# millardjn/rusty_sr

Hardware: AMD Instinct MI355X
Metric: output megapixels/sec at 3x upscale (BASELINE '4x'; reference factor is hard-wired 3) (higher is better)
Workload: dtype f32

## Files before the change

rusty_sr_amd/csrc/sr_kernels.hip:

```cpp
#include <hip/hip_runtime.h>
#include <stddef.h>
#include <stdint.h>

#include <mutex>
#include <set>
#include <type_traits>
#include <utility>

#include "sr_kernels.h"

#pragma clang fp contract(off)

typedef float f32x2 __attribute__((ext_vector_type(2)));
struct f32p { float x, y; };
__device__ __forceinline__ f32p operator+(f32p a, f32p b) { return f32p{a.x + b.x, a.y + b.y}; }
__device__ __forceinline__ f32p operator-(f32p a, f32p b) { return f32p{a.x - b.x, a.y - b.y}; }
__device__ __forceinline__ f32p operator*(f32p a, f32p b) { return f32p{a.x * b.x, a.y * b.y}; }
__device__ __forceinline__ f32p p_fma(f32p a, f32p b, f32p c) { return f32p{__builtin_fmaf(a.x, b.x, c.x), __builtin_fmaf(a.y, b.y, c.y)}; }
__device__ __forceinline__ void store_map8(char* p, uint32_t a, uint32_t b) { *(uint2*)p = make_uint2(a, b); }
typedef float f32x4 __attribute__((ext_vector_type(4)));
typedef float f32x16 __attribute__((ext_vector_type(16)));
typedef _Float16 f16x8 __attribute__((ext_vector_type(8)));
typedef _Float16 f16x2 __attribute__((ext_vector_type(2)));

template <int PREC>
constexpr bool kPlanar = PREC == 1;
template <int PREC, bool FINAL>
constexpr bool kH16 = PREC == 1 && !FINAL;

namespace {

constexpr int kThreads = 256;
constexpr int kTW = 32;
constexpr int kChunkFloats = 1024;
constexpr int kRingSlots = 5;
constexpr int kRingAhead = 4;
constexpr int kRingBytes = kRingSlots * 4096;

__device__ __forceinline__ float belu(float v, float beta) {
    return __fadd_rn(__fadd_rn(__fmul_rn(beta, v), __builtin_amdgcn_sqrtf(__fadd_rn(__fmul_rn(v, v), 1.0f))), -1.0f);
}

__device__ __forceinline__ f32x2 belu2(f32x2 v, float beta) {
    const f32x2 one = {1.0f, 1.0f};
    const f32x2 t = v * v + one;
    const f32x2 s = {__builtin_amdgcn_sqrtf(t.x), __builtin_amdgcn_sqrtf(t.y)};
    const f32x2 b = {beta, beta};
    return (b * v + s) - one;
}

__device__ __forceinline__ f32p split_value(f32p accm, f32p accx) {
    return p_fma(accx, f32p{1.0f / 2048.0f, 1.0f / 2048.0f}, accm);
}
__device__ __forceinline__ f32p belu2_fused2(f32p v, f32p beta) {
    const f32p one = {1.0f, 1.0f};
    const f32p t = p_fma(v, v, one);
    const f32p s = {__builtin_amdgcn_sqrtf(t.x), __builtin_amdgcn_sqrtf(t.y)};
    return p_fma(beta, v, s) - one;
}

__device__ __forceinline__ void store_belu_tile(float* base, const f32x16& acc, float bias, float beta) {
#pragma unroll
    for (int r = 0; r < 16; r += 2) {
        const f32x2 bb = {bias, bias};
        const f32x2 o = belu2(f32x2{acc[r], acc[r + 1]} + bb, beta);
        const int row = (r & 3) + 8 * (r >> 2);
        base[row * 32] = o.x;
        base[(row + 1) * 32] = o.y;
    }
}

__device__ __forceinline__ void store_belu_tile_lds(float* grow, float* stage, const f32x16& acc, float bias, float beta, int lane) {
    float* sp = stage + (4 * (lane >> 5)) * 32 + (lane & 31);
#pragma unroll
    for (int r = 0; r < 16; r += 2) {
        const f32x2 bb = {bias, bias};
        const f32x2 o = belu2(f32x2{acc[r], acc[r + 1]} + bb, beta);
        const int row = (r & 3) + 8 * (r >> 2);
        sp[row * 32] = o.x;
        sp[(row + 1) * 32] = o.y;
    }
    const f32x4* lp = (const f32x4*)stage + lane;
    const f32x4 v0 = lp[0], v1 = lp[64], v2 = lp[128], v3 = lp[192];
    f32x4* gp = (f32x4*)grow + lane;
    gp[0] = v0; gp[64] = v1; gp[128] = v2; gp[192] = v3;
}

__device__ __forceinline__ int xcd_remap(int bid, int nblk) {
    const int q = nblk >> 3, r = nblk & 7, xcd = bid & 7, idx = bid >> 3;
    return (xcd < r ? xcd * (q + 1) : r * (q + 1) + (xcd - r) * q) + idx;
}

__device__ __forceinline__ int tile_div(int t, TileDiv d) {
    return (int)((__umulhi((uint32_t)t, d.m) + (uint32_t)t) >> d.s);
}

__device__ __forceinline__ void tile_coords(const TileGrid& g, int tiles_x, int t, int& n, int& tx, int& ty) {
    const int tpi = tiles_x * g.tiles_y;
    n = tile_div(t, g.div_tpi);
    const int r = t - n * tpi;
    if (g.bw == 0) {
        ty = tile_div(r, g.div_tx);
        tx = r - ty * tiles_x;
    } else {
        int b = tile_div(r, g.div_blk);
        if (b > g.nfull) b = g.nfull;
        const int rr = r - b * g.bw * g.tiles_y;
        const bool full = b < g.nfull;
        const int w = full ? g.bw : tiles_x - g.nfull * g.bw;
        ty = full ? tile_div(rr, g.div_bw) : tile_div(rr, g.div_rem);
        tx = b * g.bw + (rr - ty * w);
    }
}

__device__ __forceinline__ float load_img(const void* img, int img_ch, bool u8, size_t px, int c) {
    if (u8) return __fdiv_rn((float)((const uint8_t*)img)[px * img_ch + c], 255.0f);
    return ((const float*)img)[px * 3 + c];
}

constexpr float kLoScale = 2048.0f;
typedef __fp16 fp16x2_t __attribute__((ext_vector_type(2)));

__device__ __forceinline__ void split_half2(f32p v, uint32_t& hi2, uint32_t& lo2) {
    const fp16x2_t h = __builtin_amdgcn_cvt_pkrtz(v.x, v.y);
    const f32p hf = {(float)h.x, (float)h.y};
    const f32p r = (v - hf) * f32p{kLoScale, kLoScale};
    hi2 = __builtin_bit_cast(uint32_t, h);
    lo2 = __builtin_bit_cast(uint32_t, __builtin_amdgcn_cvt_pkrtz(r.x, r.y));
}

typedef unsigned short u16x2 __attribute__((ext_vector_type(2)));
__device__ __forceinline__ void domain_track(uint32_t& dom, uint32_t hi2) {
    dom = __builtin_bit_cast(uint32_t, __builtin_elementwise_max(__builtin_bit_cast(u16x2, dom), __builtin_bit_cast(u16x2, hi2 & 0x7fff7fffu)));
}
__device__ __forceinline__ void domain_report(uint32_t dom, int* flag) {
    if (((dom & 0xffffu) >= 0x7bffu) | ((dom >> 16) >= 0x7bffu)) *(volatile int*)flag = 1;
}

__device__ __forceinline__ void store_belu_tile_split_cr(char* base, const f32x16& accm, const f32x16& accx, const f32x4 (&beta)[4], bool write,
                                                         long group_stride, long lo_off, uint32_t& dom) {
#pragma unroll
    for (int j = 0; j < 4; ++j) {
        const int r = 4 * j;
        const f32p v01 = belu2_fused2(split_value(f32p{accm[r], accm[r + 1]}, f32p{accx[r], accx[r + 1]}), f32p{beta[j][0], beta[j][1]});
        const f32p v23 = belu2_fused2(split_value(f32p{accm[r + 2], accm[r + 3]}, f32p{accx[r + 2], accx[r + 3]}), f32p{beta[j][2], beta[j][3]});
        uint32_t h01, l01, h23, l23;
        split_half2(v01, h01, l01);
        split_half2(v23, h23, l23);
        domain_track(dom, h01);
        domain_track(dom, h23);
        if (write) {
            store_map8(base + j * group_stride, h01, h23);
            store_map8(base + j * group_stride + lo_off, l01, l23);
        }
    }
}

template <typename F>
__device__ __forceinline__ void for_each_acc_row(F&& f) {
#pragma unroll
    for (int r = 0; r < 16; ++r) f(r, (r & 3) + 8 * (r >> 2));
}

}

__device__ __forceinline__ const char* uniform_ptr(const void* p) {
    const uint64_t v = (uint64_t)(uintptr_t)p;
    const uint32_t lo = __builtin_amdgcn_readfirstlane((uint32_t)v), hi = __builtin_amdgcn_readfirstlane((uint32_t)(v >> 32));
    return (const char*)(uintptr_t)(((uint64_t)hi << 32) | lo);
}

template <int TH, bool IMG_U8>
__global__ __launch_bounds__(kThreads, 2) void conv0_kernel(Conv0Args a) {
    constexpr int T = TH / 4;
    constexpr int TWH = kTW + 4, THH = TH + 4, NPIX = THH * TWH;
    __shared__ __attribute__((aligned(16))) float s_x[NPIX * 3 + 16];
    __shared__ __attribute__((aligned(16))) float s_w[5 * 8 * 64];

    const int tid = threadIdx.x, lane = tid & 63;
    const int wave = __builtin_amdgcn_readfirstlane(tid >> 6);
    const int i = lane & 31, h = lane >> 5;
    const int tiles_per_img = a.tiles_x * a.tiles_y;
    for (int k = tid; k < 5 * 8 * 64; k += kThreads) s_w[k] = a.wpack[k];
    if (tid < 16) s_x[NPIX * 3 + tid] = 0.f;
    if (blockIdx.x == 0 && tid < 40) a.queue_reset[tid] = (a.queue_grid[tid >> 3] - (tid & 7) + 7) >> 3;
    __shared__ float s_lut[256];
    if constexpr (IMG_U8) s_lut[tid] = __fdiv_rn((float)tid, 255.0f);
    const float bias = a.bias[i], beta = a.beta[i];
  for (int bid = blockIdx.x; bid < a.n_tiles; bid += gridDim.x) {
    const int n = tile_div(bid, a.div_tpi), t = bid - n * tiles_per_img;
// ... 1236 lines not shown
    f32x16 wacc[NWACC];
#pragma unroll
    for (int p = 0; p < NWACC; ++p)
#pragma unroll
        for (int r = 0; r < 16; ++r) wacc[p][r] = 0.f;
    int gtap = 0, slot = 0;
    auto taps = [&](auto ks_tag) {
        constexpr int KS = decltype(ks_tag)::value;
        if constexpr (WINO) {
            using G = TileGeom<TH, KS>;
            RingStream sm{ring, a.wpack, gtap, slot, NTAPS, wave, lane};
#pragma unroll 1
            for (int half = 0; half < 2; ++half) {
                if constexpr (KS == KS0) half_steps_wino<G::TWH, G::PLANE, T>(wacc, tile + half * 4 * G::PLANE, ring, sm, wave, lane);
                else half_steps_pairs<G::TWH, G::PLANE, T>(wacc, tile + half * 4 * G::PLANE, ring, sm, wave, lane);
            }
        } else if constexpr (H16) source_steps_h16<TH, KS, T>(qm, qx, tile, ring, a.wpack, gtap, slot, NTAPS, wave, lane);
        else source_steps<TH, KS, T, NTN, PREC>(acc, accx, tile, ring, a.wpack, gtap, slot, NTAPS, wave, lane);
    };
    ring_barrier<0>();
    __builtin_amdgcn_s_setprio(0);
    taps(std::integral_constant<int, KS0>{});
    if constexpr (NSRC >= 2) {
        __builtin_amdgcn_s_setprio(3);
        stage_tile<TH, 3, PREC, NW>(tile, a.src[1], off3, a.img_stride, a.pitch, n, y0, x0, wave, lane);
        ring_barrier<0>();
        __builtin_amdgcn_s_setprio(0);
        taps(std::integral_constant<int, 3>{});
    }
    if constexpr (NSRC >= 3) {
        __builtin_amdgcn_s_setprio(3);
        stage_tile<TH, 3, PREC, NW>(tile, a.src[2], off3, a.img_stride, a.pitch, n, y0, x0, wave, lane);
        ring_barrier<0>();
        __builtin_amdgcn_s_setprio(0);
        taps(std::integral_constant<int, 3>{});
    }
    __builtin_amdgcn_s_setprio(3);
    if constexpr (FINAL)
        lin_taps<TH, T, IMG_U8, NW * 64, NTN, PREC, FACTOR>(acc, accx, tile, ring, a, a.wpack + (size_t)NTAPS * kChunkFloats, n, y0, x0, wave, lane, tid);
    uint32_t dom = 0;
    if constexpr (WINO) {
        stage_epilogue_wino<T, NWACC>(a, wacc, bias[0], beta, n, x0, y0, wave, lane, nullptr);
    } else if constexpr (H16) {
        stage_epilogue_h16<T>(a, qm, qx, beta2, n, x0, y0, wave, lane, dom);
    } else if constexpr (FINAL && PREC == 1) {
        f32x4 fbias[NTN][4];
#pragma unroll
        for (int nt = 0; nt < NTN; ++nt)
#pragma unroll
            for (int k = 0; k < 4; ++k) fbias[nt][k] = *(const f32x4*)(a.bias + 32 * nt + 16 * (lane >> 5) + 4 * k);
        stage_epilogue_final_t<T, NTN, OUT_U8, FACTOR>(a, acc, accx, fbias, n, x0, y0, wave, lane);
    } else {
        static_assert(PREC == 0, "the split-half mode's tiles have epilogues of their own");
        stage_epilogue<TH, T, NTN, FINAL, OUT_U8, FACTOR>(a, acc, bias, beta, n, x0, y0, wave, lane);
    }
    if constexpr (PREC == 1 && !FINAL) domain_report(dom, a.domain);
}

#define SR_WAIT_ROW(k, extra) "s_waitcnt vmcnt(" #k ")" extra "\n\ts_branch .Lsrwait%=\n\t"
#define SR_WAIT_ROWS10(b, extra)                                                                                              \
    SR_WAIT_ROW(b##0, extra) SR_WAIT_ROW(b##1, extra) SR_WAIT_ROW(b##2, extra) SR_WAIT_ROW(b##3, extra) SR_WAIT_ROW(b##4, extra) \
    SR_WAIT_ROW(b##5, extra) SR_WAIT_ROW(b##6, extra) SR_WAIT_ROW(b##7, extra) SR_WAIT_ROW(b##8, extra) SR_WAIT_ROW(b##9, extra)
#define SR_WAIT_JUMP(maxn)                                                                                                   \
    "s_max_i32 %0, %1, 0\n\ts_min_i32 %0, %0, " #maxn "\n\ts_lshl_b32 %0, %0, 3\n\ts_add_u32 %0, %0, 12\n\t"                 \
    "s_getpc_b64 vcc\n\ts_add_u32 vcc_lo, vcc_lo, %0\n\ts_addc_u32 vcc_hi, vcc_hi, 0\n\ts_setpc_b64 vcc\n\t"
#define SR_WAIT_TABLE(extra)                                                                                                \
    SR_WAIT_JUMP(15) SR_WAIT_ROWS10(, extra) SR_WAIT_ROW(10, extra) SR_WAIT_ROW(11, extra) SR_WAIT_ROW(12, extra)               \
    SR_WAIT_ROW(13, extra) SR_WAIT_ROW(14, extra) SR_WAIT_ROW(15, extra) ".Lsrwait%=:"
#define SR_WAIT_TABLE64(extra)                                                                                              \
    SR_WAIT_JUMP(63) SR_WAIT_ROWS10(, extra) SR_WAIT_ROWS10(1, extra) SR_WAIT_ROWS10(2, extra) SR_WAIT_ROWS10(3, extra)         \
    SR_WAIT_ROWS10(4, extra) SR_WAIT_ROWS10(5, extra) SR_WAIT_ROW(60, extra) SR_WAIT_ROW(61, extra) SR_WAIT_ROW(62, extra)      \
    SR_WAIT_ROW(63, extra) ".Lsrwait%=:"
template <bool LGKM, bool WIDE = false>
__device__ __forceinline__ void wait_vm_n(int pending) {
    if (__builtin_constant_p(pending)) {
        switch (pending < 0 ? 0 : pending) {
#define SR_CASE(k) case k: if constexpr (LGKM) asm volatile("s_waitcnt vmcnt(" #k ") lgkmcnt(0)" ::: "memory"); else asm volatile("s_waitcnt vmcnt(" #k ")" ::: "memory"); break;
            SR_CASE(0) SR_CASE(1) SR_CASE(2) SR_CASE(3) SR_CASE(4) SR_CASE(5) SR_CASE(6) SR_CASE(7) SR_CASE(8) SR_CASE(9) SR_CASE(10)
            SR_CASE(11) SR_CASE(12) SR_CASE(13) SR_CASE(14)
#undef SR_CASE
            default: if constexpr (LGKM) asm volatile("s_waitcnt vmcnt(15) lgkmcnt(0)" ::: "memory"); else asm volatile("s_waitcnt vmcnt(15)" ::: "memory"); break;
        }
        return;
    }
    const int p = __builtin_amdgcn_readfirstlane(pending);
    int t;
    if constexpr (WIDE) {
        if constexpr (LGKM) asm volatile(SR_WAIT_TABLE64(" lgkmcnt(0)") : "=&s"(t) : "s"(p) : "vcc", "scc", "memory");
        else asm volatile(SR_WAIT_TABLE64("") : "=&s"(t) : "s"(p) : "vcc", "scc", "memory");
    } else {
        if constexpr (LGKM) asm volatile(SR_WAIT_TABLE(" lgkmcnt(0)") : "=&s"(t) : "s"(p) : "vcc", "scc", "memory");
        else asm volatile(SR_WAIT_TABLE("") : "=&s"(t) : "s"(p) : "vcc", "scc", "memory");
    }
}
template <bool LGKM, bool WIDE = false>
__device__ __forceinline__ void wait_vm_barrier(int pending) {
    wait_vm_n<LGKM, WIDE>(pending);
    __builtin_amdgcn_s_barrier();
    asm volatile("" ::: "memory");
}

template <int KS>
struct HalfTile {
    using G = TileGeom<8, KS>;
    static constexpr int NG_SMALL = TileGeom<4, KS>::NG;
    static constexpr int BYTES = 4 * G::PLANE;
    static constexpr int STEPS = (KS * KS + 1) / 2;
    static_assert(TileGeom<4, KS>::TWH == G::TWH, "a small tile is the top of a big one");
    uint32_t off[G::NG];
    template <int PREC>
    __device__ __forceinline__ void init(int pitch, int lane) {
#pragma unroll
        for (int g = 0; g < G::NG; ++g) {
            const int P = min(g * 64 + lane, G::NPIX - 1);
            const int prow = P / G::TWH, pcol = P - prow * G::TWH;
            off[g] = kPlanar<PREC> ? (uint32_t)(prow * pitch) * 128u + (uint32_t)pcol * 16u : (uint32_t)(prow * pitch + pcol) * 128u;
        }
    }
    template <int PREC>
    static __device__ __forceinline__ int chunk_of(int khalf, int wave) {
        return PREC == 0 ? 4 * khalf + wave : (wave < 2 ? 2 * khalf + wave : 4 + 2 * khalf + (wave - 2));
    }
    template <int PREC>
    __device__ __forceinline__ void stage(uint32_t buf, const float* __restrict__ src, int khalf, long img_stride, int pitch,
                                          int n, int y0, int x0, int wave) const {
        const char* origin = origin_of<PREC>(src, khalf, img_stride, pitch, n, y0, x0, wave);
        const uint32_t dst = __builtin_amdgcn_readfirstlane(buf + wave * G::PLANE);
#pragma unroll
        for (int g = 0; g < G::NG; ++g) lds_dma16<0>(origin, off[g], dst + g * 1024);
    }
    template <int PREC>
    static __device__ __forceinline__ const char* origin_of(const float* __restrict__ src, int khalf, long img_stride, int pitch, int n,
                                                            int y0, int x0, int wave) {
        if constexpr (kPlanar<PREC>)
            return uniform_ptr((const char*)(src + ((size_t)n * img_stride + (long)(y0 - G::R) * pitch) * 32) + (long)(x0 - G::R) * 16 +
                               (size_t)chunk_of<PREC>(khalf, wave) * pitch * 16);
        else
            return uniform_ptr((const char*)(src + ((size_t)n * img_stride + (long)(y0 - G::R) * pitch + (x0 - G::R)) * 32) +
                               chunk_of<PREC>(khalf, wave) * 16);
    }
    static __device__ __forceinline__ uint32_t plane_of(uint32_t buf, int wave) { return __builtin_amdgcn_readfirstlane(buf + wave * G::PLANE); }
    __device__ __forceinline__ void stage_one(int g, const char* origin, uint32_t dst) const { lds_dma16<0>(origin, off[g], dst + g * 1024); }
};

struct StepStream {
    int slot;
    int nsteps;
    bool have_next;
    int issued;
    int q[kRingAhead];
    int tile_seq;
};

__device__ __forceinline__ void step_request(StepStream& st, int gs, uint32_t ring_lds, const char* wbase, int lane) {
    int req = gs + kRingAhead;
    bool go = true;
    if (req >= st.nsteps) {
        go = st.have_next;
        req -= st.nsteps;
    }
#pragma unroll
    for (int k = 0; k + 1 < kRingAhead; ++k) st.q[k] = st.q[k + 1];
    if (go) {
        int s2 = st.slot + kRingAhead;
        if (s2 >= kRingSlots) s2 -= kRingSlots;
        lds_dma16_at(wbase, (uint32_t)req * 4096u, (uint32_t)(lane * 16), ring_lds + s2 * 4096);
        ++st.issued;
    }
    st.q[kRingAhead - 1] = st.issued;
}
template <int EXTRA>
__device__ __forceinline__ void step_advance(StepStream& st, bool tile, bool wide = false) {
    int need = st.q[EXTRA];
    if (tile && st.tile_seq > need) need = st.tile_seq;
    if (wide) wait_vm_barrier<EXTRA == 0, true>(st.issued - need);
    else wait_vm_barrier<EXTRA == 0>(st.issued - need);
    st.slot = st.slot == kRingSlots - 1 ? 0 : st.slot + 1;
}

struct HalfRequest {
    int ng;
    const char* origin;
    uint32_t dst;
};

__device__ __forceinline__ void wait_vm(int pending) { wait_vm_n<false>(pending); }

template <bool IMG_U8, int TH>
struct LinPrefetch {
    static constexpr int TWH = kTW + 2, THH = TH + 2, NPIX = THH * TWH, PER = (NPIX + 255) / 256;
    uint32_t raw[PER][3];
    int seq;
    __device__ __forceinline__ void issue(const StageArgs& a, int n, int y0, int x0, int tid, StepStream& st) {
#pragma unroll
        for (int k = 0; k < PER; ++k) {
            const int p = min(tid + 256 * k, NPIX - 1);
            const int py = p / TWH, px = p - py * TWH;
            const int gy = min(max(y0 - 1 + py, 0), a.H - 1), gx = min(max(x0 - 1 + px, 0), a.W - 1);
            const size_t gp = (size_t)n * a.H * a.W + (size_t)gy * a.W + gx;
            if constexpr (IMG_U8) {
                const uint8_t* q = (const uint8_t*)a.img + gp * a.img_ch;
                asm volatile("global_load_ubyte %0, %1, off" : "=v"(raw[k][0]) : "v"(q) : "memory");
                asm volatile("global_load_ubyte %0, %1, off offset:1" : "=v"(raw[k][1]) : "v"(q) : "memory");
                asm volatile("global_load_ubyte %0, %1, off offset:2" : "=v"(raw[k][2]) : "v"(q) : "memory");
            } else {
                const float* q = (const float*)a.img + gp * 3;
                asm volatile("global_load_dword %0, %1, off" : "=v"(raw[k][0]) : "v"(q) : "memory");
                asm volatile("global_load_dword %0, %1, off offset:4" : "=v"(raw[k][1]) : "v"(q) : "memory");
                asm volatile("global_load_dword %0, %1, off offset:8" : "=v"(raw[k][2]) : "v"(q) : "memory");
            }
        }
        st.issued += 3 * PER;
        seq = st.issued;
    }
    __device__ __forceinline__ void store_split(char* s_hi, int lo_off, const uint32_t* s_lut2, float scale, int tid, const StepStream& st) {
        wait_vm(st.issued - seq);
#pragma unroll
        for (int k = 0; k < PER; ++k)
#pragma unroll
            for (int ch = 0; ch < 3; ++ch) asm volatile("" : "+v"(raw[k][ch]));
#pragma unroll
        for (int k = 0; k < PER; ++k) {
            const int p = tid + 256 * k;
            if (p < NPIX) {
                if constexpr (IMG_U8) lin_split_store_u8(s_hi, lo_off, p, s_lut2[raw[k][0]], s_lut2[raw[k][1]], s_lut2[raw[k][2]]);
                else lin_split_store_f32(s_hi, lo_off, p, __uint_as_float(raw[k][0]), __uint_as_float(raw[k][1]), __uint_as_float(raw[k][2]), scale);
            }
        }
    }
    __device__ __forceinline__ void store(float* s_x, const float* s_lut, int tid, const StepStream& st) {
        wait_vm(st.issued - seq);
#pragma unroll
        for (int k = 0; k < PER; ++k)
#pragma unroll
            for (int ch = 0; ch < 3; ++ch) asm volatile("" : "+v"(raw[k][ch]));
#pragma unroll
        for (int k = 0; k < PER; ++k) {
            const int p = tid + 256 * k;
            if (p < NPIX) {
                f32x4 v;
                if constexpr (IMG_U8) {
                    v.x = s_lut[raw[k][0]]; v.y = s_lut[raw[k][1]]; v.z = s_lut[raw[k][2]];
                } else {
                    v.x = __uint_as_float(raw[k][0]); v.y = __uint_as_float(raw[k][1]); v.z = __uint_as_float(raw[k][2]);
                }
                v.w = 0.f;
                *(f32x4*)&s_x[p * 4] = v;
            }
        }
    }
};

struct QueueState {
    uint32_t pulled;
    uint32_t heads;
    int seq_pull, seq_snap;
    int own;
};
__device__ __forceinline__ void queue_pull_async(const StageArgs& a, int xcd, int wave, int lane, StepStream& st, QueueState& qs) {
    if (wave != 0) return;
    if (lane == 0) {
        const int* p = a.queue + xcd;
        asm volatile("global_atomic_add %0, %1, %2, off sc0" : "=v"(qs.pulled) : "v"(p), "v"(1u) : "memory");
    }
    qs.seq_pull = ++st.issued;
}
__device__ __forceinline__ void queue_presolve(const StageArgs& a, int xcd, int wave, int lane, StepStream& st, QueueState& qs) {
    if (wave != 0) return;
    wait_vm(st.issued - qs.seq_pull);
    asm volatile("" : "+v"(qs.pulled));
    const int idx = __builtin_amdgcn_readfirstlane((int)qs.pulled);
    qs.own = queue_slot(xcd, a.grid[0].ntiles, a.grid[1].ntiles, idx);
    if (qs.own < 0) {
        const int* p = a.queue + (lane & 7);
        asm volatile("global_load_dword %0, %1, off sc1" : "=v"(qs.heads) : "v"(p) : "memory");
        qs.seq_snap = ++st.issued;
    }
}
__device__ __forceinline__ void queue_publish(const StageArgs& a, int xcd, int wave, int lane, StepStream& st, QueueState& qs, volatile int* mailbox) {
    if (wave != 0) return;
    int t = qs.own;
    if (t < 0) {
        const int nbig = a.grid[0].ntiles, nsmall = a.grid[1].ntiles;
        wait_vm(st.issued - qs.seq_snap);
        asm volatile("" : "+v"(qs.heads));
        for (int k = 1; k < 8 && t < 0; ++k) {
            const int x = (xcd + k) & 7;
            if ((int)__builtin_amdgcn_readlane((int)qs.heads, x) >= queue_total(x, nbig, nsmall)) continue;
            int j = 0;
            if (lane == 0) j = atomicAdd(&a.queue[x], 1);
            t = queue_slot(x, nbig, nsmall, __builtin_amdgcn_readfirstlane(j));
        }
    }
    if (lane == 0) *mailbox = t;
    asm volatile("s_waitcnt lgkmcnt(0)" ::: "memory");
}

struct NoHook { __device__ __forceinline__ void operator()() const {} };
template <int PREC, int KSN, typename Hook = NoHook>
struct PipeStream {
    StepStream& st;
    const HalfRequest& rq;
    const HalfTile<KSN>& htn;
    const StageArgs& a;
    uint32_t ring_lds;
    const char* wbase;
    int gs0;
    int wave, lane;
    volatile int* mailbox;
    int xcd;
    QueueState& qs;
    int snap_step;
    int step_no;
    Hook last_step_hook;
    __device__ __forceinline__ void begin_step() {
        step_request(st, gs0 + step_no, ring_lds, wbase, lane);
        if (mailbox && step_no == snap_step) queue_presolve(a, xcd, wave, lane, st, qs);
        ++step_no;
    }
    __device__ __forceinline__ void piece(int g) {
        if (g < HalfTile<KSN>::G::NG && g < rq.ng) {
            htn.stage_one(g, rq.origin, rq.dst);
            st.tile_seq = ++st.issued;
        }
    }
    __device__ __forceinline__ int slot() const { return st.slot; }
    template <int EXTRA> __device__ __forceinline__ void end_step(bool last) {
        if (last) last_step_hook();
        if (last && mailbox) queue_publish(a, xcd, wave, lane, st, qs, mailbox);
        step_advance<EXTRA>(st, last, PREC == 1 && gs0 + step_no <= kRingAhead);
    }
};

template <int NSRC, int KS0, bool FINAL, bool IMG_U8, bool OUT_U8, int PREC, int FACTOR = 3, bool WINO = false>
__global__ __launch_bounds__(256, 2) void conv_stage_pipe_kernel(StageArgs a) {
    static_assert(!WINO || (NSRC <= 2 && KS0 == 5 && !FINAL && PREC == 0), "WINO: stages 1 and 2 of the exact mode");
    __builtin_amdgcn_s_setprio(3);
    constexpr int NTN = FINAL ? (FACTOR * FACTOR + 9) / 10 : 1;
    using H0 = HalfTile<KS0>;
    using H3 = HalfTile<3>;
    constexpr int HB = H0::BYTES;
    constexpr int NH = 2 * NSRC;
    constexpr bool H16 = kH16<PREC, FINAL>;
    constexpr int NSTEPS = WINO ? 2 * (kWinoSteps + (NSRC - 1) * H3::STEPS)
                         : H16 ? KS0 * KS0 + (NSRC - 1) * 9
                               : 2 * (H0::STEPS + (NSRC - 1) * H3::STEPS) * NTN;
    extern __shared__ __attribute__((aligned(16))) char smem[];
    char* ring = smem + 2 * HB;
    volatile int* s_next = (volatile int*)(ring + kRingBytes);
    float* s_wlin = (float*)(ring + kRingBytes + 16);
    float* s_lut = s_wlin + 9 * NTN * 128;
    constexpr bool kLinOwn = FINAL && NTN == 1;
    float* s_xown = s_lut + 256;
    const uint32_t lds0 = lds_addr(smem);

    const int tid = threadIdx.x, lane = tid & 63;
    const int wave = __builtin_amdgcn_readfirstlane(tid >> 6);
    const int i = lane & 31;
    const int nbig = a.grid[0].ntiles, nsmall = a.grid[1].ntiles;
    const int xcd = blockIdx.x & 7;
    const uint32_t ring_lds = __builtin_amdgcn_readfirstlane(lds_addr(ring) + wave * 1024);
    const char* wbase = uniform_ptr((const char*)a.wpack + wave * 1024);
    float bias[NTN];
#pragma unroll
    for (int nt = 0; nt < NTN; ++nt) bias[nt] = a.bias[nt * 32 + i];
    const float beta = FINAL ? 0.f : a.beta[i];
    f32x4 bias2[2], beta2[2];
#pragma unroll
    for (int ch = 0; ch < 2; ++ch) {
        bias2[ch] = H16 ? *(const f32x4*)(a.bias + 16 * ch + 4 * (lane >> 4)) : f32x4{0.f, 0.f, 0.f, 0.f};
        beta2[ch] = H16 ? *(const f32x4*)(a.beta + 16 * ch + 4 * (lane >> 4)) : f32x4{0.f, 0.f, 0.f, 0.f};
    }
    constexpr bool kFinalT = FINAL && PREC == 1;
    f32x4 fbias[kFinalT ? NTN : 1][4];
    if constexpr (kFinalT) {
#pragma unroll
        for (int nt = 0; nt < NTN; ++nt)
#pragma unroll
            for (int k = 0; k < 4; ++k) fbias[nt][k] = *(const f32x4*)(a.bias + 32 * nt + 16 * (lane >> 5) + 4 * k);
    }
    constexpr bool kQuad = FINAL && PREC == 0;
    float qbias[kQuad ? 3 * FACTOR * FACTOR : 1];
    if constexpr (kQuad) {
#pragma unroll
        for (int ch = 0; ch < 3 * FACTOR * FACTOR; ++ch) {
            const int tr = ch / 3, tl = tr % 10;
            qbias[ch] = a.bias[(tr / 10) * 32 + 16 * (tl / 5) + 3 * (tl % 5) + ch % 3];
        }
    }
    H0 h0;
    H3 h3;
    h0.template init<PREC>(a.pitch, lane);
    if constexpr (NSRC >= 2) h3.template init<PREC>(a.pitch, lane);

    typedef const uint32_t __attribute__((address_space(4)))* KernWords;
    static_assert(sizeof(TileGrid) == 64 && offsetof(StageArgs, grid) % 4 == 0, "TileGrid is read as 16 dwords");
    auto coords = [&](int t, int& n, int& x0, int& y0, bool& small) {
        KernWords kw = (KernWords)__builtin_amdgcn_kernarg_segment_ptr();
        asm volatile("" : "+s"(kw));
        int tx, ty;
        small = t >= nbig;
        uint32_t words[16];
#pragma unroll
        for (int k = 0; k < 16; ++k) words[k] = kw[offsetof(StageArgs, grid) / 4 + (small ? 16 : 0) + k];
        TileGrid g;
        __builtin_memcpy(&g, words, sizeof(g));
        tile_coords(g, a.tiles_x, small ? t - nbig : t, n, tx, ty);
        y0 = g.y0 + ty * (small ? 4 : 8);
        x0 = tx * kTW;
    };

    if constexpr (FINAL) {
        const float* wlin = a.wpack + (size_t)NSTEPS * kChunkFloats;
        for (int k = tid; k < (PREC == 1 ? 3 * NTN * 256 : 9 * NTN * 128); k += 256) s_wlin[k] = wlin[k];
        if constexpr (IMG_U8) s_lut[tid] = PREC == 1 ? __uint_as_float(lin_split_table_entry(tid, 4.0f * FACTOR * FACTOR)) : __fdiv_rn((float)tid, 255.0f);
    }
    const int first = queue_first(blockIdx.x, nbig, nsmall);
    if (first < 0) return;
    const bool single = (int)gridDim.x >= nbig + nsmall;
    int n, x0, y0;
    bool small;
    coords(first, n, x0, y0, small);
    h0.template stage<PREC>(lds0, a.src[0], 0, a.img_stride, a.pitch, n, y0, x0, wave);
#pragma unroll
    for (int k = 0; k < kRingAhead; ++k) weight_chunk_async(ring + k * 4096, a.wpack + k * kChunkFloats, wave, lane);
    constexpr int NG0 = H0::G::NG;
    StepStream st{0, NSTEPS, false, NG0 + kRingAhead, {0, NG0 + 2, NG0 + 3, NG0 + 4}, NG0};
    static_assert(kRingAhead == 4, "q[] initialiser");
    wait_vm_barrier<true>(st.issued - (NG0 + 1 + (PREC == 1 ? 1 : 0)));

    int nn = 0, nx0 = 0, ny0 = 0;
    bool nsmall_tile = false;
    uint32_t dom = 0;

    auto tile_body = [&](auto tc) {
        constexpr int T = decltype(tc)::value;
        constexpr int TH = 4 * T;
        f32x16 acc[NTN * T], accx[PREC == 1 ? NTN * T : 1];
#pragma unroll
        for (int m = 0; m < NTN * T; ++m)
#pragma unroll
            for (int r = 0; r < 16; ++r) {
                acc[m][r] = (PREC == 1 && !FINAL) ? bias[0] : 0.f;
                if constexpr (PREC == 1) accx[m][r] = 0.f;
            }
        f32x4 qm[H16 ? T : 1][2][2], qx[H16 ? T : 1][2][2];
        if constexpr (H16) {
#pragma unroll
            for (int m = 0; m < T; ++m)
#pragma unroll
                for (int k = 0; k < 4; ++k) { qm[m][k >> 1][k & 1] = bias2[k & 1]; qx[m][k >> 1][k & 1] = f32x4{0.f, 0.f, 0.f, 0.f}; }
        }
        constexpr bool QUAD = FINAL && PREC == 0 && T == 2;
        QuadAcc qa[QUAD ? NTN : 1];
        if constexpr (QUAD) {
#pragma unroll
            for (int nt = 0; nt < NTN; ++nt)
#pragma unroll
                for (int g = 0; g < 8; ++g) qa[nt][g] = f32x4{0.f, 0.f, 0.f, 0.f};
        }
        constexpr int NWACC = WINO ? 3 + NSRC : 1;
        f32x16 wacc[NWACC];
#pragma unroll
        for (int p = 0; p < NWACC; ++p)
#pragma unroll
            for (int r = 0; r < 16; ++r) wacc[p][r] = 0.f;
        QueueState qs{0u, 0u, 0, 0, -1};
        if (!single) queue_pull_async(a, xcd, wave, lane, st, qs);
        st.have_next = false;
        LinPrefetch<IMG_U8, TH> linpx;
        auto do_half = [&](auto jc) {
            constexpr int j = decltype(jc)::value;
            constexpr int src = j >> 1;
            constexpr int KSJ = src == 0 ? KS0 : 3;
            constexpr int KSN = (j + 1 < NH) ? (((j + 1) >> 1) == 0 ? KS0 : 3) : KS0;
            const uint32_t other = lds0 + ((j + 1) & 1) * HB;
            const char* hb = smem + (j & 1) * HB;
            if constexpr (j == 1) {
                const int next = single ? -1 : __builtin_amdgcn_readfirstlane(*s_next);
                st.have_next = next >= 0;
                if (st.have_next) coords(next, nn, nx0, ny0, nsmall_tile);
            }
            HalfRequest rq;
            if constexpr (j + 1 < NH)
                rq = HalfRequest{T == 2 ? HalfTile<KSN>::G::NG : HalfTile<KSN>::NG_SMALL,
                                 HalfTile<KSN>::template origin_of<PREC>(a.src[(j + 1) >> 1], (j + 1) & 1, a.img_stride, a.pitch, n, y0, x0, wave),
                                 HalfTile<KSN>::plane_of(other, wave)};
            else
                rq = HalfRequest{!st.have_next ? 0 : nsmall_tile ? HalfTile<KSN>::NG_SMALL : HalfTile<KSN>::G::NG,
                                 HalfTile<KSN>::template origin_of<PREC>(a.src[0], 0, a.img_stride, a.pitch, nn, ny0, nx0, wave),
                                 HalfTile<KSN>::plane_of(other, wave)};
            if constexpr (FINAL && j == (kLinOwn ? NH - 2 : NH - 1)) linpx.issue(a, n, y0, x0, tid, st);
            const HalfTile<KSN>* htn;
            if constexpr (KSN == KS0) htn = (const HalfTile<KSN>*)&h0; else htn = (const HalfTile<KSN>*)&h3;
            using GJ = TileGeom<8, KSJ>;
            constexpr int PAIRS_J = (KSJ * KSJ - 1) / 2;
            constexpr int STEPS_J = WINO ? (src == 0 ? kWinoSteps : H3::STEPS) : H16 ? PAIRS_J + (j & 1) : HalfTile<KSJ>::STEPS * NTN;
            constexpr int GS0 = WINO ? (j < 2 ? j * kWinoSteps : 2 * kWinoSteps + (j - 2) * H3::STEPS) : H16 ? (src == 0 ? 0 : KS0 * KS0 + (src - 1) * 9) + (j & 1) * PAIRS_J
                                    : (j == 0 ? 0 : j == 1 ? H0::STEPS : 2 * H0::STEPS + (j - 2) * H3::STEPS) * NTN;
            constexpr int LIN_LO_J = LinPrefetch<IMG_U8, TH>::NPIX * 8;
            auto lin_store = [&]() {
                if constexpr (kLinOwn && j == NH - 2) {
                    if constexpr (PREC == 1) linpx.store_split((char*)s_xown, LIN_LO_J, (const uint32_t*)s_lut, 4.0f * FACTOR * FACTOR, tid, st);
                    else linpx.store(s_xown, s_lut, tid, st);
                    asm volatile("s_waitcnt lgkmcnt(0)" ::: "memory");
                }
            };
            PipeStream<PREC, KSN, decltype(lin_store)> sm{st, rq, *htn, a, ring_lds, wbase, GS0, wave, lane, (j == 0 && !single) ? s_next : nullptr, xcd, qs, STEPS_J > 3 ? STEPS_J - 3 : 0, 0, lin_store};
            if constexpr (WINO && src == 0) half_steps_wino<GJ::TWH, GJ::PLANE, T>(wacc, hb, ring, sm, wave, lane);
            else if constexpr (WINO) half_steps_pairs<GJ::TWH, GJ::PLANE, T>(wacc, hb, ring, sm, wave, lane);
            else if constexpr (QUAD) half_steps_f32<GJ::TWH, GJ::PLANE, KSJ, T, NTN, true, FACTOR>(qa, hb, ring, sm, wave, lane);
            else if constexpr (PREC == 0) half_steps_f32<GJ::TWH, GJ::PLANE, KSJ, T, NTN>(acc, hb, ring, sm, wave, lane);
            else if constexpr (H16) half_steps_h16<GJ::TWH, GJ::PLANE, 2, KSJ, T, (j & 1) != 0, -HB>(qm, qx, hb, ring, sm, wave, lane);
            else half_steps_h<GJ::TWH, GJ::PLANE, 2, KSJ, T, NTN>(acc, accx, hb, ring, sm, wave, lane);
        };
        do_half(std::integral_constant<int, 0>{});
        do_half(std::integral_constant<int, 1>{});
        if constexpr (NH > 2) { do_half(std::integral_constant<int, 2>{}); do_half(std::integral_constant<int, 3>{}); }
        if constexpr (NH > 4) { do_half(std::integral_constant<int, 4>{}); do_half(std::integral_constant<int, 5>{}); }
        if constexpr (FINAL) {
            constexpr int LIN_LO = LinPrefetch<IMG_U8, TH>::NPIX * 8;
            float* s_x = kLinOwn ? s_xown : (float*)(smem + HB);
            if constexpr (!kLinOwn) {
                if constexpr (PREC == 1) linpx.store_split((char*)s_x, LIN_LO, (const uint32_t*)s_lut, 4.0f * FACTOR * FACTOR, tid, st);
                else linpx.store(s_x, s_lut, tid, st);
                asm volatile("s_waitcnt lgkmcnt(0)" ::: "memory");
                __builtin_amdgcn_s_barrier();
                asm volatile("" ::: "memory");
            }
            if constexpr (PREC == 1) lin_mfma_h<TH, T, NTN>(acc, accx, (const char*)s_x, LIN_LO, (const f16x8*)s_wlin, wave, lane);
            else if constexpr (QUAD) lin_mfma_quad<NTN, FACTOR>(qa, s_x, s_wlin, wave, lane);
            else lin_mfma<TH, T, NTN>(acc, s_x, s_wlin, wave, lane);
            if constexpr (!kLinOwn) {
                asm volatile("s_waitcnt lgkmcnt(0)" ::: "memory");
                __builtin_amdgcn_s_barrier();
                asm volatile("" ::: "memory");
            }
        }
        int stores;
        if constexpr (H16) stores = stage_epilogue_h16<T>(a, qm, qx, beta2, n, x0, y0, wave, lane, dom);
        else if constexpr (QUAD) stores = stage_epilogue_quad<NTN, OUT_U8, FACTOR>(a, qa, qbias, n, x0, y0, wave, lane);
        else if constexpr (kFinalT) stores = stage_epilogue_final_t<T, NTN, OUT_U8, FACTOR>(a, acc, accx, fbias, n, x0, y0, wave, lane);
        else {
            float* scratch = FINAL ? nullptr : (float*)(smem + ((NH - 1) & 1) * HB + wave * H0::G::PLANE);
            if constexpr (WINO) stores = stage_epilogue_wino<T, NWACC>(a, wacc, bias[0], beta, n, x0, y0, wave, lane, scratch);
            else stores = stage_epilogue<TH, T, NTN, FINAL, OUT_U8, FACTOR>(a, acc, bias, beta, n, x0, y0, wave, lane, scratch);
        }
        if constexpr (PREC == 1) st.issued += stores;
    };

    constexpr bool kBigTiles = !(FINAL && FACTOR == 4 && PREC == 1);
    int budget = nbig + nsmall;
    while (true) {
        if constexpr (kBigTiles) {
            if (small) tile_body(std::integral_constant<int, 1>{});
            else tile_body(std::integral_constant<int, 2>{});
        } else {
            if (!small) __builtin_trap();
            tile_body(std::integral_constant<int, 1>{});
        }
        if (!st.have_next) break;
        if (--budget <= 0) {
            asm volatile("s_waitcnt vmcnt(0)" ::: "memory");
            __builtin_trap();
        }
        n = nn; x0 = nx0; y0 = ny0; small = nsmall_tile;
    }
    if constexpr (PREC == 1 && !FINAL) domain_report(dom, a.domain);
}


__global__ __launch_bounds__(256) void clear_borders_kernel(ClearArgs a) {
    float4* m = reinterpret_cast<float4*>(a.map[blockIdx.y]);
    const long rows_per = a.img_stride / a.pitch;
    const long row = blockIdx.x;
    const long base = row * a.pitch;
    long end = base + a.pitch;
    if (end > a.total_px) end = a.total_px;
    const long img = row / rows_per, local = row - img * rows_per;
    const bool interior = img < a.n && local >= kFeatPad && local < kFeatPad + a.H;
    const float4 z = make_float4(0.f, 0.f, 0.f, 0.f);
    if (!interior) {
        for (long q = base * 8 + threadIdx.x; q < end * 8; q += 256) m[q] = z;
        return;
    }
    if (a.planar) {
        const int edge = kFeatPad + (a.pitch - kFeatPad - a.W);
        for (int k = threadIdx.x; k < 8 * edge; k += 256) {
            const int c = k / edge, e = k - c * edge;
            m[base * 8 + (long)c * a.pitch + (e < kFeatPad ? e : a.W + e)] = z;
        }
        return;
    }
    for (long q = base * 8 + threadIdx.x; q < (base + kFeatPad) * 8; q += 256) m[q] = z;
    for (long q = (base + kFeatPad + a.W) * 8 + threadIdx.x; q < end * 8; q += 256) m[q] = z;
}

hipError_t sr_launch_clear_borders(const ClearArgs& a, hipStream_t s) {
    const long rows = (a.total_px + a.pitch - 1) / a.pitch;
    hipLaunchKernelGGL(clear_borders_kernel, dim3((unsigned)rows, 4), dim3(256), 0, s, a);
    return hipGetLastError();
}

template <int TH, int KS0>
static constexpr size_t stage_lds_bytes() {
    return 8 * (size_t)TileGeom<TH, KS0>::PLANE + kRingBytes;
}

template <int TH>
static hipError_t launch_conv0_t(const Conv0Args& a, int nblk, bool img_u8, hipStream_t s) {
    if (img_u8)
        hipLaunchKernelGGL((conv0_kernel<TH, true>), dim3(nblk), dim3(kThreads), 0, s, a);
    else
        hipLaunchKernelGGL((conv0_kernel<TH, false>), dim3(nblk), dim3(kThreads), 0, s, a);
    return hipGetLastError();
}

template <int TH>
static hipError_t launch_conv0_split_t(const Conv0Args& a, int nblk, bool img_u8, hipStream_t s) {
    if (img_u8)
        hipLaunchKernelGGL((conv0_split_kernel<TH, true>), dim3(nblk), dim3(kThreads), 0, s, a);
    else
        hipLaunchKernelGGL((conv0_split_kernel<TH, false>), dim3(nblk), dim3(kThreads), 0, s, a);
    return hipGetLastError();
}

hipError_t sr_launch_conv0(const Conv0Args& a, int th, int prec, int nblk, bool img_u8, hipStream_t s) {
    if (prec == 0) return th == 8 ? launch_conv0_t<8>(a, nblk, img_u8, s) : launch_conv0_t<4>(a, nblk, img_u8, s);
    return th == 8 ? launch_conv0_split_t<8>(a, nblk, img_u8, s) : launch_conv0_split_t<4>(a, nblk, img_u8, s);
}

template <typename K>
static hipError_t launch_with_lds(K kern, const StageArgs& a, int nblk, size_t lds, hipStream_t s) {
    static std::mutex mu;
    static std::set<std::pair<const void*, int>> configured;
    int dev = 0;
    hipError_t e = hipGetDevice(&dev);
    if (e != hipSuccess) return e;
    {
        std::lock_guard<std::mutex> lock(mu);
        const auto key = std::make_pair((const void*)kern, dev);
        if (!configured.count(key)) {
            e = hipFuncSetAttribute((const void*)kern, hipFuncAttributeMaxDynamicSharedMemorySize, (int)lds);
            if (e != hipSuccess) return e;
            configured.insert(key);
        }
    }
    hipLaunchKernelGGL(kern, dim3(nblk), dim3(kThreads), lds, s, a);
    return hipGetLastError();
}

template <int TH, int PREC>
static hipError_t launch_stage_t(int stage, int factor, const StageArgs& a, int nblk, bool img_u8, bool out_u8, bool wino,
                                 hipStream_t s) {
    switch (stage) {
        case 1:
            if constexpr (PREC == 0)
                if (wino) return launch_with_lds(conv_stage_kernel<TH, 1, 5, false, false, false, 0, 3, true>, a, nblk, stage_lds_bytes<TH, 5>(), s);
            return launch_with_lds(conv_stage_kernel<TH, 1, 5, false, false, false, PREC>, a, nblk, stage_lds_bytes<TH, 5>(), s);
        case 2:
            if constexpr (PREC == 0)
// ... 61 lines not shown
```

Measured before the change: 5304.

## Pair weight-ring barriers in final f32 stage with shallower prefetch

For the final stage in exact (PREC 0) mode, the weight-chunk ring now prefetches three steps ahead instead of four. This frees one slot so two consecutive steps can share a single wait-plus-barrier, and the step advance skips the barrier on even steps. The aim is to halve the workgroup barrier count in the final conv stage's weight streaming loop. In exchange, less prefetch distance is available to hide global-to-LDS latency, and the ring bookkeeping becomes more intricate.

```diff
diff --git a/rusty_sr_amd/csrc/sr_kernels.hip b/rusty_sr_amd/csrc/sr_kernels.hip
--- a/rusty_sr_amd/csrc/sr_kernels.hip
+++ b/rusty_sr_amd/csrc/sr_kernels.hip
@@ -36,6 +36,9 @@
 constexpr int kRingSlots = 5;
 constexpr int kRingAhead = 4;
 constexpr int kRingBytes = kRingSlots * 4096;
+#ifndef SR_PAIR_BARRIERS
+#define SR_PAIR_BARRIERS 1
+#endif
 
 __device__ __forceinline__ float belu(float v, float beta) {
     return __fadd_rn(__fadd_rn(__fmul_rn(beta, v), __builtin_amdgcn_sqrtf(__fadd_rn(__fmul_rn(v, v), 1.0f))), -1.0f);
@@ -1578,22 +1581,24 @@
     int tile_seq;
 };
 
+template <int AHEAD = kRingAhead>
 __device__ __forceinline__ void step_request(StepStream& st, int gs, uint32_t ring_lds, const char* wbase, int lane) {
-    int req = gs + kRingAhead;
+    static_assert(AHEAD >= 1 && AHEAD <= kRingAhead, "");
+    int req = gs + AHEAD;
     bool go = true;
     if (req >= st.nsteps) {
         go = st.have_next;
         req -= st.nsteps;
     }
 #pragma unroll
-    for (int k = 0; k + 1 < kRingAhead; ++k) st.q[k] = st.q[k + 1];
+    for (int k = 0; k + 1 < AHEAD; ++k) st.q[k] = st.q[k + 1];
     if (go) {
-        int s2 = st.slot + kRingAhead;
+        int s2 = st.slot + AHEAD;
         if (s2 >= kRingSlots) s2 -= kRingSlots;
         lds_dma16_at(wbase, (uint32_t)req * 4096u, (uint32_t)(lane * 16), ring_lds + s2 * 4096);
         ++st.issued;
     }
-    st.q[kRingAhead - 1] = st.issued;
+    st.q[AHEAD - 1] = st.issued;
 }
 template <int EXTRA>
 __device__ __forceinline__ void step_advance(StepStream& st, bool tile, bool wide = false) {
@@ -1723,7 +1728,7 @@
 }
 
 struct NoHook { __device__ __forceinline__ void operator()() const {} };
-template <int PREC, int KSN, typename Hook = NoHook>
+template <int PREC, int KSN, typename Hook = NoHook, bool PAIRS = false>
 struct PipeStream {
     StepStream& st;
     const HalfRequest& rq;
@@ -1739,8 +1744,9 @@
     int snap_step;
     int step_no;
     Hook last_step_hook;
+    int nsteps_half;
     __device__ __forceinline__ void begin_step() {
-        step_request(st, gs0 + step_no, ring_lds, wbase, lane);
+        step_request<PAIRS ? 3 : kRingAhead>(st, gs0 + step_no, ring_lds, wbase, lane);
         if (mailbox && step_no == snap_step) queue_presolve(a, xcd, wave, lane, st, qs);
         ++step_no;
     }
@@ -1754,6 +1760,20 @@
     template <int EXTRA> __device__ __forceinline__ void end_step(bool last) {
         if (last) last_step_hook();
         if (last && mailbox) queue_publish(a, xcd, wave, lane, st, qs, mailbox);
+        if constexpr (PAIRS) {
+            static_assert(PREC == 0, "");
+            const int l = step_no - 1;
+            if (!last && (l & 1) == 0) {
+                st.slot = st.slot == kRingSlots - 1 ? 0 : st.slot + 1;
+                return;
+            }
+            const bool two = last || l + 2 < nsteps_half;
+            int need = two ? st.q[1] : st.q[0];
+            if (last && st.tile_seq > need) need = st.tile_seq;
+            wait_vm_barrier<true>(st.issued - need);
+            st.slot = st.slot == kRingSlots - 1 ? 0 : st.slot + 1;
+            return;
+        }
         step_advance<EXTRA>(st, last, PREC == 1 && gs0 + step_no <= kRingAhead);
     }
 };
@@ -1841,6 +1861,8 @@
         for (int k = tid; k < (PREC == 1 ? 3 * NTN * 256 : 9 * NTN * 128); k += 256) s_wlin[k] = wlin[k];
         if constexpr (IMG_U8) s_lut[tid] = PREC == 1 ? __uint_as_float(lin_split_table_entry(tid, 4.0f * FACTOR * FACTOR)) : __fdiv_rn((float)tid, 255.0f);
     }
+    constexpr bool kPairBarriers = FINAL && PREC == 0 && SR_PAIR_BARRIERS;
+    constexpr int kAhead = kPairBarriers ? 3 : kRingAhead;
     const int first = queue_first(blockIdx.x, nbig, nsmall);
     if (first < 0) return;
     const bool single = (int)gridDim.x >= nbig + nsmall;
@@ -1849,11 +1871,11 @@
     coords(first, n, x0, y0, small);
     h0.template stage<PREC>(lds0, a.src[0], 0, a.img_stride, a.pitch, n, y0, x0, wave);
 #pragma unroll
-    for (int k = 0; k < kRingAhead; ++k) weight_chunk_async(ring + k * 4096, a.wpack + k * kChunkFloats, wave, lane);
+    for (int k = 0; k < kAhead; ++k) weight_chunk_async(ring + k * 4096, a.wpack + k * kChunkFloats, wave, lane);
     constexpr int NG0 = H0::G::NG;
-    StepStream st{0, NSTEPS, false, NG0 + kRingAhead, {0, NG0 + 2, NG0 + 3, NG0 + 4}, NG0};
+    StepStream st{0, NSTEPS, false, NG0 + kAhead, {0, NG0 + 2, NG0 + 3, NG0 + 4}, NG0};
     static_assert(kRingAhead == 4, "q[] initialiser");
-    wait_vm_barrier<true>(st.issued - (NG0 + 1 + (PREC == 1 ? 1 : 0)));
+    wait_vm_barrier<true>(st.issued - (NG0 + 1 + (PREC == 1 || kPairBarriers ? 1 : 0)));
 
     int nn = 0, nx0 = 0, ny0 = 0;
     bool nsmall_tile = false;
@@ -1932,7 +1954,8 @@
                     asm volatile("s_waitcnt lgkmcnt(0)" ::: "memory");
                 }
             };
-            PipeStream<PREC, KSN, decltype(lin_store)> sm{st, rq, *htn, a, ring_lds, wbase, GS0, wave, lane, (j == 0 && !single) ? s_next : nullptr, xcd, qs, STEPS_J > 3 ? STEPS_J - 3 : 0, 0, lin_store};
+            PipeStream<PREC, KSN, decltype(lin_store), kPairBarriers> sm{st, rq, *htn, a, ring_lds, wbase, GS0, wave, lane, (j == 0 && !single) ? s_next : nullptr, xcd, qs,
+                                                                         STEPS_J > 3 ? STEPS_J - 3 : 0, 0, lin_store, STEPS_J};
             if constexpr (WINO && src == 0) half_steps_wino<GJ::TWH, GJ::PLANE, T>(wacc, hb, ring, sm, wave, lane);
             else if constexpr (WINO) half_steps_pairs<GJ::TWH, GJ::PLANE, T>(wacc, hb, ring, sm, wave, lane);
             else if constexpr (QUAD) half_steps_f32<GJ::TWH, GJ::PLANE, KSJ, T, NTN, true, FACTOR>(qa, hb, ring, sm, wave, lane);
```

After: 5315 (median of 6 runs). No clear change (+0.2%).
